# Hiroshiba/realtime-yukarin

Hardware: NVIDIA H100
Metric: chunks_per_s_0.3s_24kHz_encode_stage1_stage2_vocode (higher is better)
Workload: dtype f64 (WORLD analysis / synthesis, SPTK), f16 operands / f32 accumulate: stage-2 k4 layers on wgmma, stage-1 k4 layers on mma.sync inside the one-launch cluster kernel; f32 CUDA cores (3x3 / k3 edge layers)

## Files before the change

### realtime_yukarin_b200/csrc/api.cu

```cuda
#include <math.h>
#include <stddef.h>
#include <stdlib.h>
#include <string.h>
#include <mutex>
#include <algorithm>
#include <vector>

#include "../../include/ryk.h"
#include "conv.h"
#include "drift.h"
#include "engine.h"
#include "fft.cuh"
#include "features.h"
#include "synth.h"
#include "unet.h"

namespace ryk {

static thread_local std::string g_err;
void set_error(const std::string& msg) { g_err = msg; }

void fft_fill_twiddles(double2* t) {
  for (int k = 0; k < kTwiddleN / 2; ++k) t[k] = make_double2(cos(2.0 * kPi * k / kTwiddleN), -sin(2.0 * kPi * k / kTwiddleN));
}
// ... 109 lines not shown
  if (voiced[i]) v = has_stats ? (float)exp((log((double)f0[i]) - mu_i) / sd_i * sd_t + mu_t) : f0[i];
  out[i] = v;
}

static int stage1_plan_for(Engine* e, int Tp, UNetPlan** plan) {
  RYK_CHECK(e->voices[0]->stage1 != nullptr, "stage-1 model not loaded");
  return unet_get_plan(e, e->voices[0]->stage1, 1, 1, Tp, e->precision, plan);
}
static int stage2_plan_for(Engine* e, int Tp, UNetPlan** plan) {
  RYK_CHECK(e->voices[0]->stage2 != nullptr, "stage-2 model not loaded");
  return unet_get_plan(e, e->voices[0]->stage2, 1, Tp, 512, e->precision, plan);
}

static int voice_for_update(Engine* e, int id, Voice** out) {
  Voice* v = engine_voice(e, id);
  RYK_CHECK(v != nullptr, "no such voice");
  RYK_CHECK(id == 0 || v->users == 0, "voice is in use by a session or group: destroy them before changing its models or statistics");
  *out = v;
  return 0;
}

}

using namespace ryk;

static Engine* E(ryk_engine* e) { return &e->impl; }

extern "C" {

int ryk_abi_version(void) { return 1; }
const char* ryk_last_error(void) { return g_err.c_str(); }

int ryk_engine_create(int device, ryk_engine** out) {
  RYK_CHECK(out != nullptr, "null out pointer");
  setenv("CUDA_DEVICE_MAX_CONNECTIONS", "32", 0);
  int count = 0;
  RYK_CUDA(cudaGetDeviceCount(&count));
  RYK_CHECK(count > 0 && device < count, "no such CUDA device (libryk has no CPU fallback)");
  RYK_CUDA(cudaSetDevice(device));
  cudaDeviceProp prop;
  RYK_CUDA(cudaGetDeviceProperties(&prop, device));
  RYK_CHECK(prop.major == 9 && prop.minor == 0, "libryk is built for sm_90a (H100) only");
  ryk_engine* h = new ryk_engine();
  Engine* e = &h->impl;
  e->device = device;
  e->voices.push_back(new Voice());
  RYK_CUDA(cudaStreamCreateWithFlags(&e->stream, cudaStreamNonBlocking));
  std::vector<double2> tw(kTwiddleN / 2);
  fft_fill_twiddles(tw.data());
  RYK_CUDA(cudaMalloc(&e->d_twiddle, sizeof(double2) * tw.size()));
  RYK_CUDA(cudaMemcpy(e->d_twiddle, tw.data(), sizeof(double2) * tw.size(), cudaMemcpyHostToDevice));
  if (analysis_kernels_init()) return -1;
  if (tc_init()) return -1;
  if (s1_fused_init()) return -1;
  RYK_CUDA(cudaMalloc(&e->d_colmin, sizeof(float) * kColminFloats));
  RYK_CUDA(cudaMalloc(&e->d_launches, sizeof(*e->d_launches)));
  RYK_CUDA(cudaMemset(e->d_launches, 0, sizeof(*e->d_launches)));
  *out = h;
  return 0;
}

int ryk_engine_destroy(ryk_engine* h) {
  if (!h) return 0;
  Engine* e = E(h);
  cudaSetDevice(e->device);
  cudaStreamSynchronize(e->stream);
  drift_destroy_all(e);
  reblock_destroy_all(e);
  session_destroy_all(e);
  crepe_destroy();
  for (auto& kv : e->dio_plans) dio_plan_free(kv.second);
  for (Voice* v : e->voices) voice_free(v);
  for (Synth* s : e->synths) synth_destroy(s);
  for (auto& kv : e->sptk) { cudaFree(kv.second.d_G); cudaFree(kv.second.d_H); }
  void* ptrs[] = {e->d_colmin, e->d_launches, e->d_twiddle, e->d_jump, e->d_scratch};
  for (void* p : ptrs) if (p) cudaFree(p);
  if (e->h_pinned) cudaFreeHost(e->h_pinned);
  cudaStreamDestroy(e->stream);
  delete h;
  return 0;
}

int ryk_engine_set_precision(ryk_engine* h, int mode) {
  RYK_CHECK(mode == 0 || mode == 1, "precision mode must be 0 (fp32) or 1 (fp16 tensor core)");
  E(h)->precision = mode;
  return 0;
}
int ryk_engine_get_precision(ryk_engine* h) { return E(h)->precision; }
int ryk_engine_set_stage1_fused(ryk_engine* h, int enable) { E(h)->s1_fused = enable != 0; return s1_fused_cluster_size(); }
long long ryk_engine_launch_count(ryk_engine* h) {
  Engine* e = E(h);
  unsigned long long device_count = 0;
  RYK_CUDA(cudaSetDevice(e->device));
  RYK_CUDA(cudaDeviceSynchronize());
  RYK_CUDA(cudaMemcpy(&device_count, e->d_launches, sizeof(device_count), cudaMemcpyDeviceToHost));
  return e->launches + (long long)device_count;
}
int ryk_engine_synchronize(ryk_engine* h) { RYK_CUDA(cudaSetDevice(E(h)->device)); RYK_CUDA(cudaDeviceSynchronize()); return 0; }

int ryk_engine_profile(ryk_engine* h, int enable) { E(h)->profile = enable != 0; return 0; }
int ryk_engine_profile_read2(ryk_engine* h, double* stage2_ms_total, double* stage2_ms_union, int* stage2_runs) {
  Engine* e = E(h);
  RYK_CUDA(cudaDeviceSynchronize());
  double tot = 0.0, uni = 0.0;
  std::vector<std::pair<double, double>> iv;
  for (auto& pr : e->prof_events) {
// ... 693 lines not shown
```

### realtime_yukarin_b200/csrc/conv.h

```cpp
#pragma once
#include <cuda.h>

#include "common.cuh"

namespace ryk {

enum Act { ACT_NONE = 0, ACT_LEAKY = 1, ACT_RELU = 2 };
enum DType { DT_F32 = 0, DT_F16 = 1 };

constexpr int kMaxGroupVoices = 8;
constexpr int kMaxGroupBatch = 64;

struct LayerWeights {
  const float* w[kMaxGroupVoices];
  const float* scale[kMaxGroupVoices];
  const float* shift[kMaxGroupVoices];
  float host_scale[kMaxGroupVoices], host_shift[kMaxGroupVoices];
  uint8_t voice_of[kMaxGroupBatch];
};
__host__ __device__ inline int item_voice(const LayerWeights& wt, int b) { return b < kMaxGroupBatch ? wt.voice_of[b] : 0; }
struct TcWeightMaps { CUtensorMap m[kMaxGroupVoices]; };

struct ConvLayer {
  int transposed = 0;
  int B = 1, Hin = 1, Win = 1, Hout = 1, Wout = 1;
  int C0 = 0, C1 = 0, Cout = 0;
  int KH = 1, KW = 1, SH = 1, SW = 1, PH = 0, PW = 0;
  int act = ACT_NONE;
  int band_y0 = 0, band_y1 = 0;
  int skip_y0 = 0, skip_y1 = 0;
  int run_y0 = 0, run_y1 = 0;
  const void* in0 = nullptr; const void* in1 = nullptr; int in_dtype = DT_F32;
  void* out = nullptr; int out_dtype = DT_F32;
  int n_voices = 1;
  LayerWeights wt = {};
  bool host_scale_valid = false;
  const __half* w_tc[kMaxGroupVoices] = {};
  const __half* w_frag = nullptr;
  int ksplit = 1;
  int ksplit_tiles = 0;
  CUtensorMap tmA0, tmA1, tmO;
  TcWeightMaps tmB;
  int tile_w = 0, tile_h = 0;
  int block_n = 0;
  bool tc_ready = false;
};

inline int layer_class_rows(const ConvLayer& L) { return L.transposed ? L.Hin : L.Hout; }
inline int layer_band_end(const ConvLayer& L) { return L.band_y1 > 0 ? L.band_y1 : layer_class_rows(L); }
inline void layer_band_out_rows(const ConvLayer& L, int* r0, int* r1) {
  const int s = L.transposed ? L.SH : 1;
  *r0 = L.band_y0 * s;
  *r1 = layer_band_end(L) * s < L.Hout ? layer_band_end(L) * s : L.Hout;
}

int pack_weights_direct(const float* d_w_chainer, int transposed, int Cin, int Cout, int KH, int KW, float* d_out, cudaStream_t st);
int pack_weights_tc(const float* d_w_chainer, int transposed, int Cin, int Cout, int KH, int KW, int SH, int SW, __half* d_out, cudaStream_t st);

int conv_direct_run(const ConvLayer& L, cudaStream_t st);
bool conv_direct_band_supported(const ConvLayer& L);
bool conv_direct_cin1(const ConvLayer& L);
constexpr int kCin1Rows = 8;
bool conv_direct_per_item_weights(const ConvLayer& L);

bool tc_layer_eligible(const ConvLayer& L);
int tc_init();
int tc_layer_prepare(ConvLayer& L, int num_sms);
int tc_layer_weight_maps(ConvLayer& L);
int conv_tc_run(const ConvLayer& L, cudaStream_t st);
int tc_tile_rows(const ConvLayer& L);
int tc_tile_count(const ConvLayer& L);

int s1_pack_weights(const float* d_w_chainer, int transposed, int Cin, int Cout, __half* d_out, cudaStream_t st);
int s1_fused_init();
int s1_fused_cluster_size();

}
```

### realtime_yukarin_b200/csrc/conv_direct.cu

```cuda
#include "conv.h"

namespace ryk {

template <typename T> __device__ inline float ld_act(const T* p);
template <> __device__ inline float ld_act<float>(const float* p) { return *p; }
template <> __device__ inline float ld_act<__half>(const __half* p) { return __half2float(*p); }
template <typename T> __device__ inline void st_act(T* p, float v);
template <> __device__ inline void st_act<float>(float* p, float v) { *p = v; }
template <> __device__ inline void st_act<__half>(__half* p, float v) { *p = __float2half_rn(v); }

struct DirectParams {
  int transposed, B, Hin, Win, Hout, Wout, C0, C1, Cout, KH, KW, SH, SW, PH, PW, act;
  int classH, classW;
  int Hc, Wc;
  const void* in0; const void* in1; void* out;
  const float* w; const float* scale; const float* shift;
};

template <typename TIn, typename TOut>
__global__ void __launch_bounds__(256) k_conv_direct(DirectParams p) {
  constexpr int BM = 64, BN = 64, BK = 16;
  __shared__ float As[BK][BM + 4];
  __shared__ float Bs[BK][BN + 4];
  __shared__ int pix_b[BM], pix_y[BM], pix_x[BM];
  const int Cin = p.C0 + p.C1;
  const int cls = blockIdx.z;
  const int py = cls / p.classW, px = cls % p.classW;
  const int npix = p.B * p.Hc * p.Wc;
  const int m0 = blockIdx.x * BM, n0 = blockIdx.y * BN;
  const int tid = threadIdx.x, ty = tid >> 4, tx = tid & 15;
  if (tid < BM) {
    int q = m0 + tid;
    if (q < npix) {
      int b = q / (p.Hc * p.Wc);
      int r = q - b * p.Hc * p.Wc;
      int my = r / p.Wc, mx = r - my * p.Wc;
      pix_b[tid] = b; pix_y[tid] = my * p.classH + py; pix_x[tid] = mx * p.classW + px;
    } else {
      pix_b[tid] = -1; pix_y[tid] = 0; pix_x[tid] = 0;
    }
  }
  __syncthreads();
  float acc[4][4];
#pragma unroll
  for (int i = 0; i < 4; ++i)
#pragma unroll
    for (int j = 0; j < 4; ++j) acc[i][j] = 0.f;

  const int a_pix = tid >> 2, a_c4 = (tid & 3) * 4;
  const int b_k = tid >> 4, b_n4 = (tid & 15) * 4;
  const TIn* in0 = (const TIn*)p.in0;
  const TIn* in1 = (const TIn*)p.in1;

// ... 39 lines not shown
#pragma unroll
          for (int i = 0; i < 4; ++i)
#pragma unroll
            for (int j = 0; j < 4; ++j) acc[i][j] = fmaf(a[i], b[j], acc[i][j]);
        }
        __syncthreads();
      }
    }
  }
  TOut* out = (TOut*)p.out;
#pragma unroll
  for (int i = 0; i < 4; ++i) {
    int pl = ty * 4 + i;
    int b = pix_b[pl];
    if (b < 0) continue;
    size_t obase = ((size_t)(b * p.Hout + pix_y[pl]) * p.Wout + pix_x[pl]) * p.Cout;
#pragma unroll
    for (int j = 0; j < 4; ++j) {
      int n = n0 + tx * 4 + j;
      if (n >= p.Cout) continue;
      float v = acc[i][j] * p.scale[n] + p.shift[n];
      if (p.act == ACT_LEAKY) v = v > 0.f ? v : 0.2f * v;
      else if (p.act == ACT_RELU) v = v > 0.f ? v : 0.f;
      st_act<TOut>(out + obase + n, v);
    }
  }
}

static int conv_direct_generic(const ConvLayer& L, cudaStream_t st) {
  DirectParams p;
  p.transposed = L.transposed; p.B = L.B; p.Hin = L.Hin; p.Win = L.Win; p.Hout = L.Hout; p.Wout = L.Wout;
  p.C0 = L.C0; p.C1 = L.C1; p.Cout = L.Cout; p.KH = L.KH; p.KW = L.KW; p.SH = L.SH; p.SW = L.SW; p.PH = L.PH; p.PW = L.PW;
  p.act = L.act;
  p.classH = L.transposed ? L.SH : 1; p.classW = L.transposed ? L.SW : 1;
  RYK_CHECK(L.Hout % p.classH == 0 && L.Wout % p.classW == 0, "transposed conv output must be a multiple of the stride");
  p.Hc = L.Hout / p.classH; p.Wc = L.Wout / p.classW;
  p.in0 = L.in0; p.in1 = L.in1; p.out = L.out; p.w = L.wt.w[0]; p.scale = L.wt.scale[0]; p.shift = L.wt.shift[0];
  RYK_CHECK(p.w && p.scale && p.shift && L.in0 && L.out, "direct conv layer is missing a device pointer");
  int npix = L.B * p.Hc * p.Wc;
  dim3 grid((npix + 63) / 64, (L.Cout + 63) / 64, p.classH * p.classW);
  if (L.in_dtype == DT_F32 && L.out_dtype == DT_F32) k_conv_direct<float, float><<<grid, 256, 0, st>>>(p);
  else if (L.in_dtype == DT_F32 && L.out_dtype == DT_F16) k_conv_direct<float, __half><<<grid, 256, 0, st>>>(p);
  else if (L.in_dtype == DT_F16 && L.out_dtype == DT_F16) k_conv_direct<__half, __half><<<grid, 256, 0, st>>>(p);
  else k_conv_direct<__half, float><<<grid, 256, 0, st>>>(p);
  RYK_CUDA(cudaGetLastError());
  return 0;
}



template <typename TOut>
__global__ void __launch_bounds__(256) k_conv3x3_cin1(const float* __restrict__ in, const __grid_constant__ LayerWeights wt, int act,
                                                     int B, int H, int W, int Cout, int skip_b0, int skip_nb, TOut* __restrict__ out) {
  constexpr int kRows = kCin1Rows;
  const int groups = Cout >> 3;
  const int g = threadIdx.x % groups, xl = threadIdx.x / groups;
  const int x = blockIdx.x * 32 + xl;
  const int y0 = (blockIdx.y + (blockIdx.y >= skip_b0 ? skip_nb : 0)) * kRows;
  const int b = blockIdx.z;
  const int voice = item_voice(wt, b);
  const float* __restrict__ w = wt.w[voice];
  const float* __restrict__ scale = wt.scale[voice];
  const float* __restrict__ shift = wt.shift[voice];
  float wr[9][8], sc[8], sh[8];
#pragma unroll
  for (int t = 0; t < 9; ++t)
#pragma unroll
    for (int j = 0; j < 8; ++j) wr[t][j] = __ldg(w + t * Cout + g * 8 + j);
#pragma unroll
  for (int j = 0; j < 8; ++j) { sc[j] = __ldg(scale + g * 8 + j); sh[j] = __ldg(shift + g * 8 + j); }
  if (x >= W) return;
  const float* base = in + (size_t)b * H * W;
  auto ld = [&](int yy, int xx) -> float { return (yy >= 0 && yy < H && xx >= 0 && xx < W) ? __ldg(base + (size_t)yy * W + xx) : 0.f; };
  float r0[3], r1[3], r2[3];
#pragma unroll
  for (int d = 0; d < 3; ++d) { r0[d] = ld(y0 - 1, x + d - 1); r1[d] = ld(y0, x + d - 1); }
  for (int yy = 0; yy < kRows; ++yy) {
    const int y = y0 + yy;
    if (y >= H) break;
#pragma unroll
    for (int d = 0; d < 3; ++d) r2[d] = ld(y + 1, x + d - 1);
    float o[8];
#pragma unroll
    for (int j = 0; j < 8; ++j) {
      float a = 0.f;
#pragma unroll
      for (int d = 0; d < 3; ++d) { a = fmaf(r0[d], wr[d][j], a); a = fmaf(r1[d], wr[3 + d][j], a); a = fmaf(r2[d], wr[6 + d][j], a); }
      a = a * sc[j] + sh[j];
      if (act == ACT_LEAKY) a = a > 0.f ? a : 0.2f * a; else if (act == ACT_RELU) a = fmaxf(a, 0.f);
      o[j] = a;
    }
    TOut* dst = out + (((size_t)b * H + y) * W + x) * Cout + g * 8;
    if constexpr (sizeof(TOut) == 2) {
      __half2 h0 = __floats2half2_rn(o[0], o[1]), h1 = __floats2half2_rn(o[2], o[3]), h2 = __floats2half2_rn(o[4], o[5]), h3 = __floats2half2_rn(o[6], o[7]);
      *reinterpret_cast<uint4*>(dst) = make_uint4(*reinterpret_cast<uint32_t*>(&h0), *reinterpret_cast<uint32_t*>(&h1),
                                                  *reinterpret_cast<uint32_t*>(&h2), *reinterpret_cast<uint32_t*>(&h3));
    } else {
      *reinterpret_cast<float4*>(dst) = make_float4(o[0], o[1], o[2], o[3]);
      *reinterpret_cast<float4*>(dst + 4) = make_float4(o[4], o[5], o[6], o[7]);
    }
#pragma unroll
    for (int d = 0; d < 3; ++d) { r0[d] = r1[d]; r1[d] = r2[d]; }
  }
}

__global__ void __launch_bounds__(256) k_conv3x3_cout1_h(const __half* __restrict__ in0, const __half* __restrict__ in1,
                                                        const __grid_constant__ LayerWeights weights, int act,
                                                        int B, int H, int W, int y0, float* __restrict__ out) {
  const int lane = threadIdx.x & 31, warp = threadIdx.x >> 5;
  const int x0 = (blockIdx.x * 8 + warp) * 8;
  const int y = y0 + blockIdx.y, b = blockIdx.z;
  const int voice = item_voice(weights, b);
  const float* __restrict__ w = weights.w[voice];
  const float scale = weights.host_scale[voice], shift = weights.host_shift[voice];
  if (x0 >= W) return;
  const __half* src = lane < 16 ? in0 : in1;
  const int c = (lane & 15) * 4;
  float wt[9][4];
#pragma unroll
  for (int t = 0; t < 9; ++t)
#pragma unroll
    for (int j = 0; j < 4; ++j) wt[t][j] = __ldg(w + t * 128 + (lane < 16 ? 0 : 64) + c + j);
  float acc[8];
#pragma unroll
  for (int q = 0; q < 8; ++q) acc[q] = 0.f;
#pragma unroll
  for (int dy = 0; dy < 3; ++dy) {
    const int iy = y + dy - 1;
    if (iy < 0 || iy >= H) continue;
    uint2 raw[10];
#pragma unroll
    for (int i = 0; i < 10; ++i) {
      const int ix = x0 + i - 1;
      raw[i] = (ix >= 0 && ix < W) ? __ldg(reinterpret_cast<const uint2*>(src + (((size_t)b * H + iy) * W + ix) * 64 + c)) : make_uint2(0u, 0u);
    }
#pragma unroll
    for (int i = 0; i < 10; ++i) {
      const float2 f01 = __half22float2(*reinterpret_cast<__half2*>(&raw[i].x)), f23 = __half22float2(*reinterpret_cast<__half2*>(&raw[i].y));
#pragma unroll
      for (int dx = 0; dx < 3; ++dx) {
        const int q = i - dx;
        if (q < 0 || q >= 8) continue;
        const float* wv = wt[dy * 3 + dx];
        acc[q] = fmaf(f01.x, wv[0], acc[q]); acc[q] = fmaf(f01.y, wv[1], acc[q]);
        acc[q] = fmaf(f23.x, wv[2], acc[q]); acc[q] = fmaf(f23.y, wv[3], acc[q]);
      }
    }
  }
#pragma unroll
  for (int q = 0; q < 8; ++q) {
#pragma unroll
    for (int o = 16; o > 0; o >>= 1) acc[q] += __shfl_xor_sync(0xffffffffu, acc[q], o);
  }
  if (lane < 8) {
    float a = acc[0];
#pragma unroll
    for (int q = 1; q < 8; ++q) a = lane == q ? acc[q] : a;
    const int x = x0 + lane;
    if (x < W) {
      a = a * scale + shift;
      if (act == ACT_LEAKY) a = a > 0.f ? a : 0.2f * a; else if (act == ACT_RELU) a = fmaxf(a, 0.f);
      out[((size_t)b * H + y) * W + x] = a;
    }
  }
}

__global__ void __launch_bounds__(256) k_conv1d_k3_small(const __half* __restrict__ in0, const __half* __restrict__ in1,
                                                        const float* __restrict__ w , const float* __restrict__ scale,
                                                        const float* __restrict__ shift, int act, int B, int W, int Cout, float* __restrict__ out) {
  const int lane = threadIdx.x & 31;
  const int pos = blockIdx.x * 8 + (threadIdx.x >> 5);
  if (pos >= B * W) return;
  const int b = pos / W, x = pos - b * W;
  const __half* src = lane < 16 ? in0 : in1;
  const int c = (lane & 15) * 4, cg = lane * 4;
  float xin[3][4];
#pragma unroll
  for (int t = 0; t < 3; ++t) {
    const int ix = x + t - 1;
    uint2 raw = make_uint2(0u, 0u);
    if (ix >= 0 && ix < W) raw = __ldg(reinterpret_cast<const uint2*>(src + ((size_t)b * W + ix) * 64 + c));
    const float2 f01 = __half22float2(*reinterpret_cast<__half2*>(&raw.x)), f23 = __half22float2(*reinterpret_cast<__half2*>(&raw.y));
    xin[t][0] = f01.x; xin[t][1] = f01.y; xin[t][2] = f23.x; xin[t][3] = f23.y;
  }
  float mine = 0.f;
  for (int co = 0; co < Cout; ++co) {
    float a = 0.f;
#pragma unroll
    for (int t = 0; t < 3; ++t)
#pragma unroll
      for (int j = 0; j < 4; ++j) a = fmaf(xin[t][j], __ldg(w + ((size_t)t * 128 + cg + j) * Cout + co), a);
#pragma unroll
    for (int o = 16; o > 0; o >>= 1) a += __shfl_xor_sync(0xffffffffu, a, o);
    if (lane == co) mine = a;
  }
  if (lane < Cout) {
    float a = mine * __ldg(scale + lane) + __ldg(shift + lane);
    if (act == ACT_LEAKY) a = a > 0.f ? a : 0.2f * a; else if (act == ACT_RELU) a = fmaxf(a, 0.f);
    out[(size_t)pos * Cout + lane] = a;
  }
}

__global__ void k_read2(const float* a, const float* b, float* out) { out[0] = a[0]; out[1] = b[0]; }

bool conv_direct_band_supported(const ConvLayer& L) {
  return !L.transposed && L.KH == 3 && L.KW == 3 && L.SH == 1 && L.SW == 1 && L.PH == 1 && L.PW == 1 && L.Cout == 1 && L.C0 == 64 &&
         L.C1 == 64 && L.in_dtype == DT_F16 && L.out_dtype == DT_F32 && L.host_scale_valid;
}

bool conv_direct_cin1(const ConvLayer& L) {
  return !L.transposed && L.KH == 3 && L.KW == 3 && L.SH == 1 && L.SW == 1 && L.PH == 1 && L.PW == 1 && L.C0 == 1 && L.C1 == 0 &&
         L.in_dtype == DT_F32 && L.Cout % 8 == 0 && L.Cout <= 64;
}

bool conv_direct_per_item_weights(const ConvLayer& L) { return conv_direct_cin1(L) || conv_direct_band_supported(L); }

int conv_direct_run(const ConvLayer& L, cudaStream_t st) {
  const bool cout1_h = conv_direct_band_supported(L);
  const bool cin1 = conv_direct_cin1(L);
  RYK_CHECK(L.n_voices == 1 || cout1_h || cin1, "of the CUDA-core kernels only the stage-2 edge layers take weights per batch item");
  RYK_CHECK(cout1_h || (L.band_y0 == 0 && L.band_y1 == 0), "of the CUDA-core kernels only the Cout = 1 3x3 kernel computes a row band");
  RYK_CHECK(cin1 || L.skip_y1 == 0, "of the CUDA-core kernels only the Cin = 1 3x3 kernel skips a padded tail");
  if (!L.transposed && L.KH == 3 && L.KW == 3 && L.SH == 1 && L.SW == 1 && L.PH == 1 && L.PW == 1) {
    if (cin1) {
      RYK_CHECK(L.skip_y0 % kCin1Rows == 0 && L.skip_y1 % kCin1Rows == 0 && L.skip_y0 <= L.skip_y1 && L.skip_y1 <= L.Hout,
                "skipped rows are not whole row blocks of the first layer");
      const int skip_b0 = L.skip_y0 / kCin1Rows, skip_nb = (L.skip_y1 - L.skip_y0) / kCin1Rows;
      dim3 grid((L.Win + 31) / 32, (L.Hin + kCin1Rows - 1) / kCin1Rows - skip_nb, L.B);
      int threads = 32 * (L.Cout / 8);
      if (L.out_dtype == DT_F16)
        k_conv3x3_cin1<__half><<<grid, threads, 0, st>>>((const float*)L.in0, L.wt, L.act, L.B, L.Hin, L.Win, L.Cout, skip_b0, skip_nb, (__half*)L.out);
      else
        k_conv3x3_cin1<float><<<grid, threads, 0, st>>>((const float*)L.in0, L.wt, L.act, L.B, L.Hin, L.Win, L.Cout, skip_b0, skip_nb, (float*)L.out);
      RYK_CUDA(cudaGetLastError());
      return 0;
    }
    if (cout1_h) {
      dim3 blocks((L.Win + 63) / 64, layer_band_end(L) - L.band_y0, L.B);
      k_conv3x3_cout1_h<<<blocks, 256, 0, st>>>((const __half*)L.in0, (const __half*)L.in1, L.wt, L.act,
                                                L.B, L.Hin, L.Win, L.band_y0, (float*)L.out);
      RYK_CUDA(cudaGetLastError());
      return 0;
    }
  }
  if (!L.transposed && L.KH == 1 && L.KW == 3 && L.SW == 1 && L.PW == 1 && L.Hin == 1 && L.C0 == 64 && L.C1 == 64 && L.Cout <= 16 &&
      L.in_dtype == DT_F16 && L.out_dtype == DT_F32) {
    const int npos = L.B * L.Win;
    k_conv1d_k3_small<<<(npos + 7) / 8, 256, 0, st>>>((const __half*)L.in0, (const __half*)L.in1, L.wt.w[0], L.wt.scale[0], L.wt.shift[0], L.act, L.B, L.Win, L.Cout,
                                                     (float*)L.out);
    RYK_CUDA(cudaGetLastError());
    return 0;
  }
  return conv_direct_generic(L, st);
}

__global__ void k_pack_direct(const float* __restrict__ w, int transposed, int Cin, int Cout, int KH, int KW, float* __restrict__ out) {
  size_t total = (size_t)KH * KW * Cin * Cout;
  for (size_t i = blockIdx.x * (size_t)blockDim.x + threadIdx.x; i < total; i += (size_t)gridDim.x * blockDim.x) {
    int n = i % Cout; size_t r = i / Cout;
    int c = r % Cin; r /= Cin;
    int kx = r % KW; int ky = r / KW;
    size_t src = transposed ? (((size_t)c * Cout + n) * KH + ky) * KW + kx : (((size_t)n * Cin + c) * KH + ky) * KW + kx;
    out[i] = w[src];
  }
}

int pack_weights_direct(const float* d_w, int transposed, int Cin, int Cout, int KH, int KW, float* d_out, cudaStream_t st) {
  k_pack_direct<<<256, 256, 0, st>>>(d_w, transposed, Cin, Cout, KH, KW, d_out);
  RYK_CUDA(cudaGetLastError());
  return 0;
}

__global__ void k_pack_tc(const float* __restrict__ w, int transposed, int Cin, int Cout, int KH, int KW, int SH, int SW,
                          __half* __restrict__ out) {
  size_t total = (size_t)KH * KW * Cin * Cout;
  for (size_t i = blockIdx.x * (size_t)blockDim.x + threadIdx.x; i < total; i += (size_t)gridDim.x * blockDim.x) {
    if (!transposed) {
      size_t K = (size_t)KH * KW * Cin;
      int n = i / K; size_t k = i % K;
      int tap = k / Cin, c = k % Cin;
      int ky = tap / KW, kx = tap % KW;
      out[i] = __float2half_rn(w[(((size_t)n * Cin + c) * KH + ky) * KW + kx]);
    } else {
      int th = KH / SH, tw = KW / SW;
      size_t K = (size_t)th * tw * Cin;
      size_t per_cls = K * Cout;
      int cls = i / per_cls; size_t r = i % per_cls;
      int n = r / K; size_t k = r % K;
      int tap = k / Cin, c = k % Cin;
      int dy = tap / tw, dx = tap % tw, py = cls / SW, px = cls % SW;
      int ky = SH == 2 ? 3 - 2 * dy - py : 0, kx = SW == 2 ? 3 - 2 * dx - px : 0;
      out[i] = __float2half_rn(w[(((size_t)c * Cout + n) * KH + ky) * KW + kx]);
    }
// ... 11 lines not shown
```

### realtime_yukarin_b200/csrc/conv_tc.cu

```cuda
#include <cuda.h>
#include <cudaTypedefs.h>

#include "conv.h"
#include "tc_ptx.cuh"

namespace ryk {

struct TcParams {
  int transposed, B, Hout, Wout, Cout;
  int Hc, Wc;
  int tile_w, tile_h, tiles_w, tiles_h;
  int th0;
  int skip_t0, skip_tn;
  int run_y0, run_y1;
  int chunks0, chunks1;
  int taps_w, ntaps;
  int sh, sw, ph, pw;
  int classes_w;
  int ksplit, chunks_per_split;
  int act;
  LayerWeights wt;
  __half* out;
};

// ... 294 lines not shown

static void tc_geometry(const ConvLayer& L, int num_sms, int* tile_w, int* tile_h, int* block_n, int* ksplit) {
  int tw, th;
  tc_tile_shape(L, &tw, &th);
  int bn = L.Cout >= 128 ? 128 : 64;
  int tiles = L.ksplit_tiles > 0 ? L.ksplit_tiles : tc_tile_count(L);
  int ntaps = L.transposed ? (L.KH / L.SH) * (L.KW / L.SW) : L.KH * L.KW;
  int total_chunks = ntaps * (L.C0 + L.C1) / kBlockK;
  int ks = 1;
  int slots = num_sms * 2;
  if (tiles < slots) {
    constexpr int kMinChunks = 8;
    ks = slots / tiles;
    if (ks > total_chunks / kMinChunks) ks = total_chunks / kMinChunks;
    if (ks > kMaxSplits) ks = kMaxSplits;
    if (ks < 1) ks = 1;
    while (ks > 1 && tiles > g_clusters[ks]) --ks;
    int cps = (total_chunks + ks - 1) / ks;
    ks = (total_chunks + cps - 1) / cps;
  }
  *tile_w = tw; *tile_h = th; *block_n = bn; *ksplit = ks;
}

int tc_layer_weight_maps(ConvLayer& L) {
  RYK_CHECK(L.n_voices >= 1 && L.n_voices <= kMaxGroupVoices, "a layer holds 1..8 voices");
  const int classes = L.transposed ? L.SH * L.SW : 1;
  const int ntaps = L.transposed ? (L.KH / L.SH) * (L.KW / L.SW) : L.KH * L.KW;
  const size_t K = (size_t)ntaps * (L.C0 + L.C1), rows = (size_t)classes * L.Cout;
  for (int v = 0; v < L.n_voices; ++v) {
    RYK_CHECK(L.w_tc[v] != nullptr, "tensor-core layer without packed weights for one of its voices");
    if (make_weight_map(&L.tmB.m[v], L.w_tc[v], K, rows, L.block_n)) return -1;
  }
  for (int v = L.n_voices; v < kMaxGroupVoices; ++v) L.tmB.m[v] = L.tmB.m[0];
  return 0;
}

int tc_layer_prepare(ConvLayer& L, int num_sms) {
  RYK_CHECK(g_encode != nullptr, "tc_init() was not called");
  RYK_CHECK(tc_layer_eligible(L), "layer is not eligible for the tensor-core path");
  tc_geometry(L, num_sms, &L.tile_w, &L.tile_h, &L.block_n, &L.ksplit);
  int stw = L.transposed ? 1 : L.SW, sth = L.transposed ? 1 : L.SH;
  if (make_act_map(&L.tmA0, L.in0, L.C0, L.Win, L.Hin, L.B, L.tile_w, L.tile_h, stw, sth)) return -1;
  if (L.C1 > 0) { if (make_act_map(&L.tmA1, L.in1, L.C1, L.Win, L.Hin, L.B, L.tile_w, L.tile_h, stw, sth)) return -1; }
  else L.tmA1 = L.tmA0;
  if (tc_layer_weight_maps(L)) return -1;
  if (make_act_map(&L.tmO, L.out, L.Cout, L.Wout, L.Hout, L.B, L.tile_w, L.tile_h, L.transposed ? L.SW : 1, L.transposed ? L.SH : 1)) return -1;
  RYK_CHECK(L.band_y0 >= 0 && L.band_y0 % L.tile_h == 0 && L.band_y0 < layer_band_end(L) && layer_band_end(L) <= layer_class_rows(L) &&
            (layer_band_end(L) % L.tile_h == 0 || layer_band_end(L) == layer_class_rows(L)), "row band is not a range of whole tile rows");
  RYK_CHECK(L.skip_y1 == 0 || (!L.transposed && L.skip_y0 % L.tile_h == 0 && L.skip_y1 % L.tile_h == 0 && L.band_y0 <= L.skip_y0 &&
                               L.skip_y0 < L.skip_y1 && L.skip_y1 <= layer_band_end(L)),
            "skipped rows are not a range of whole tile rows inside the band of a convolution");
  L.tc_ready = true;
  return 0;
}

template <typename... KArgs, typename... Args>
static cudaError_t launch_pdl(void (*kernel)(KArgs...), dim3 grid, dim3 block, size_t smem, cudaStream_t st, int cluster_z, Args&&... args) {
  cudaLaunchConfig_t cfg = {};
  cfg.gridDim = grid; cfg.blockDim = block; cfg.dynamicSmemBytes = smem; cfg.stream = st;
  cudaLaunchAttribute attr[2];
  attr[0].id = cudaLaunchAttributeProgrammaticStreamSerialization; attr[0].val.programmaticStreamSerializationAllowed = 1;
  attr[1].id = cudaLaunchAttributeClusterDimension; attr[1].val.clusterDim.x = 1; attr[1].val.clusterDim.y = 1; attr[1].val.clusterDim.z = cluster_z;
  cfg.attrs = attr; cfg.numAttrs = cluster_z > 1 ? 2 : 1;
  return cudaLaunchKernelEx(&cfg, kernel, static_cast<KArgs>(args)...);
}

int conv_tc_run(const ConvLayer& L, cudaStream_t st) {
  RYK_CHECK(L.tc_ready, "tc layer not prepared");
  TcParams p;
  p.transposed = L.transposed; p.B = L.B; p.Hout = L.Hout; p.Wout = L.Wout; p.Cout = L.Cout;
  p.Hc = L.transposed ? L.Hin : L.Hout; p.Wc = L.transposed ? L.Win : L.Wout;
  p.tile_w = L.tile_w; p.tile_h = L.tile_h;
  p.skip_t0 = L.skip_y0 / L.tile_h; p.skip_tn = (L.skip_y1 - L.skip_y0) / L.tile_h;
  p.tiles_w = (p.Wc + L.tile_w - 1) / L.tile_w; p.tiles_h = (layer_band_end(L) - L.band_y0 + L.tile_h - 1) / L.tile_h - p.skip_tn;
  p.th0 = L.band_y0 / L.tile_h;
  p.run_y0 = L.run_y0; p.run_y1 = L.run_y1;
  p.chunks0 = L.C0 / kBlockK; p.chunks1 = L.C1 / kBlockK;
  p.taps_w = L.transposed ? L.KW / L.SW : L.KW;
  p.ntaps = L.transposed ? (L.KH / L.SH) * (L.KW / L.SW) : L.KH * L.KW;
  p.sh = L.SH; p.sw = L.SW; p.ph = L.PH; p.pw = L.PW;
  p.classes_w = L.transposed ? L.SW : 1;
  const int classes = L.transposed ? L.SH * L.SW : 1;
  p.ksplit = L.ksplit;
  int total_chunks = p.ntaps * (p.chunks0 + p.chunks1);
  p.chunks_per_split = (total_chunks + L.ksplit - 1) / L.ksplit;
  p.act = L.act; p.wt = L.wt;
  p.out = (__half*)L.out;
  dim3 grid(L.B * p.tiles_w * p.tiles_h, L.Cout / L.block_n, classes * L.ksplit);
  if (L.block_n == 128) RYK_CUDA(launch_pdl(RYK_TC_N128, grid, dim3(kTcThreads), tc_smem_bytes<128, 3>(), st, L.ksplit, L.tmA0, L.tmA1, L.tmB, L.tmO, p));
  else RYK_CUDA(launch_pdl(RYK_TC_N64, grid, dim3(kTcThreads), tc_smem_bytes<64, 4>(), st, L.ksplit, L.tmA0, L.tmA1, L.tmB, L.tmO, p));
  RYK_CUDA(cudaGetLastError());
  return 0;
}

}
```

### realtime_yukarin_b200/csrc/tc_ptx.cuh

```cuda
#pragma once
#include <cuda.h>
#include <stdint.h>

namespace ryk {

constexpr int kBlockM = 128;
constexpr int kBlockK = 64;
constexpr int kMmaK = 16;
constexpr int kTcConsumers = 256;
constexpr int kTcThreads = kTcConsumers + 32;

__device__ __forceinline__ uint32_t smem_u32(const void* p) { return (uint32_t)__cvta_generic_to_shared(p); }

__device__ __forceinline__ void pdl_trigger() { asm volatile("griddepcontrol.launch_dependents;" ::: "memory"); }
__device__ __forceinline__ void pdl_wait() { asm volatile("griddepcontrol.wait;" ::: "memory"); }

__device__ __forceinline__ bool elect_one() {
  uint32_t pred;
  asm volatile("{\n\t.reg .pred p;\n\telect.sync _|p, 0xffffffff;\n\tselp.u32 %0, 1, 0, p;\n\t}" : "=r"(pred));
  return pred != 0;
}

__device__ __forceinline__ void mbar_init(uint64_t* bar, uint32_t count) {
  asm volatile("mbarrier.init.shared::cta.b64 [%0], %1;" ::"r"(smem_u32(bar)), "r"(count));
}
__device__ __forceinline__ void mbar_expect_tx(uint64_t* bar, uint32_t bytes) {
  asm volatile("mbarrier.arrive.expect_tx.shared::cta.b64 _, [%0], %1;" ::"r"(smem_u32(bar)), "r"(bytes) : "memory");
}
__device__ __forceinline__ void mbar_arrive(uint64_t* bar) {
  asm volatile("mbarrier.arrive.shared::cta.b64 _, [%0];" ::"r"(smem_u32(bar)) : "memory");
}
__device__ __forceinline__ void mbar_wait(uint64_t* bar, uint32_t parity) {
  asm volatile(
      "{\n\t"
      ".reg .pred p;\n\t"
      "WAIT_LOOP:\n\t"
      "mbarrier.try_wait.parity.shared::cta.b64 p, [%0], %1;\n\t"
      "@p bra WAIT_DONE;\n\t"
      "bra WAIT_LOOP;\n\t"
      "WAIT_DONE:\n\t"
      "}" ::"r"(smem_u32(bar)), "r"(parity) : "memory");
}
__device__ __forceinline__ void tma_load_4d(void* dst, const CUtensorMap* map, uint64_t* bar, int c0, int c1, int c2, int c3) {
  asm volatile(
      "cp.async.bulk.tensor.4d.shared::cluster.global.mbarrier::complete_tx::bytes [%0], [%1, {%3, %4, %5, %6}], [%2];"
      ::"r"(smem_u32(dst)), "l"(map), "r"(smem_u32(bar)), "r"(c0), "r"(c1), "r"(c2), "r"(c3) : "memory");
}
__device__ __forceinline__ void tma_load_2d(void* dst, const CUtensorMap* map, uint64_t* bar, int c0, int c1) {
  asm volatile(
      "cp.async.bulk.tensor.2d.shared::cluster.global.mbarrier::complete_tx::bytes [%0], [%1, {%3, %4}], [%2];"
      ::"r"(smem_u32(dst)), "l"(map), "r"(smem_u32(bar)), "r"(c0), "r"(c1) : "memory");
}
__device__ __forceinline__ void wgmma_fence() { asm volatile("wgmma.fence.sync.aligned;" ::: "memory"); }
__device__ __forceinline__ void wgmma_commit() { asm volatile("wgmma.commit_group.sync.aligned;" ::: "memory"); }
template <int N> __device__ __forceinline__ void wgmma_wait() { asm volatile("wgmma.wait_group.sync.aligned %0;" ::"n"(N) : "memory"); }
template <int R> __device__ __forceinline__ void wgmma_fence_acc(float (&d)[R]) {
#pragma unroll
  for (int i = 0; i < R; ++i) asm volatile("" : "+f"(d[i])::"memory");
}
__device__ __forceinline__ void wgmma_m64n64(float (&d)[32], uint64_t adesc, uint64_t bdesc) {
  asm volatile(
      "{\n\t.reg .pred p;\n\tsetp.ne.b32 p, %34, 0;\n\t"
      "wgmma.mma_async.sync.aligned.m64n64k16.f32.f16.f16 "
      "{%0, %1, %2, %3, %4, %5, %6, %7, %8, %9, %10, %11, %12, %13, %14, %15, %16, %17, %18, %19, %20, %21, %22, %23, %24, %25, %26, %27, %28, %29, %30, %31}, "
      "%32, %33, p, 1, 1, 0, 0;\n\t}"
      : "+f"(d[0]), "+f"(d[1]), "+f"(d[2]), "+f"(d[3]), "+f"(d[4]), "+f"(d[5]), "+f"(d[6]), "+f"(d[7]), "+f"(d[8]), "+f"(d[9]), "+f"(d[10]), "+f"(d[11]), "+f"(d[12]), "+f"(d[13]), "+f"(d[14]), "+f"(d[15]), "+f"(d[16]), "+f"(d[17]), "+f"(d[18]), "+f"(d[19]), "+f"(d[20]), "+f"(d[21]), "+f"(d[22]), "+f"(d[23]), "+f"(d[24]), "+f"(d[25]), "+f"(d[26]), "+f"(d[27]), "+f"(d[28]), "+f"(d[29]), "+f"(d[30]), "+f"(d[31])
      : "l"(adesc), "l"(bdesc), "r"(1));
}
// ... 36 lines not shown
```

Baseline: 2614.

## Launch edge 3x3 convs with PDL and stage their inputs in shared memory

The first (Cin=1) and last (Cout=1) 3x3 direct-conv kernels are now launched with programmatic dependent launch. They trigger dependents early and wait only after loading weights, so they can overlap with the previous kernel's tail. Both kernels now stage their input halo tile in shared memory: the cin1 kernel through a plain load loop, the cout1 kernel through cp.async into dynamic smem. The cout1 kernel also handles four output rows per block instead of one, reusing the staged rows across the vertical taps. This trades repeated global loads for a larger shared-memory footprint and fewer blocks.

After: 2649, median of 6. +1.4%, better.

```diff
diff --git a/realtime_yukarin_b200/csrc/api.cu b/realtime_yukarin_b200/csrc/api.cu
--- a/realtime_yukarin_b200/csrc/api.cu
+++ b/realtime_yukarin_b200/csrc/api.cu
@@ -185,6 +185,7 @@
   RYK_CUDA(cudaMemcpy(e->d_twiddle, tw.data(), sizeof(double2) * tw.size(), cudaMemcpyHostToDevice));
   if (analysis_kernels_init()) return -1;
   if (tc_init()) return -1;
+  if (conv_direct_init()) return -1;
   if (s1_fused_init()) return -1;
   RYK_CUDA(cudaMalloc(&e->d_colmin, sizeof(float) * kColminFloats));
   RYK_CUDA(cudaMalloc(&e->d_launches, sizeof(*e->d_launches)));
diff --git a/realtime_yukarin_b200/csrc/conv.h b/realtime_yukarin_b200/csrc/conv.h
--- a/realtime_yukarin_b200/csrc/conv.h
+++ b/realtime_yukarin_b200/csrc/conv.h
@@ -57,6 +57,7 @@
 int pack_weights_direct(const float* d_w_chainer, int transposed, int Cin, int Cout, int KH, int KW, float* d_out, cudaStream_t st);
 int pack_weights_tc(const float* d_w_chainer, int transposed, int Cin, int Cout, int KH, int KW, int SH, int SW, __half* d_out, cudaStream_t st);
 
+int conv_direct_init();
 int conv_direct_run(const ConvLayer& L, cudaStream_t st);
 bool conv_direct_band_supported(const ConvLayer& L);
 bool conv_direct_cin1(const ConvLayer& L);
diff --git a/realtime_yukarin_b200/csrc/conv_direct.cu b/realtime_yukarin_b200/csrc/conv_direct.cu
--- a/realtime_yukarin_b200/csrc/conv_direct.cu
+++ b/realtime_yukarin_b200/csrc/conv_direct.cu
@@ -1,4 +1,5 @@
 #include "conv.h"
+#include "pdl.cuh"
 
 namespace ryk {
 
@@ -144,10 +145,11 @@
 template <typename TOut>
 __global__ void __launch_bounds__(256) k_conv3x3_cin1(const float* __restrict__ in, const __grid_constant__ LayerWeights wt, int act,
                                                      int B, int H, int W, int Cout, int skip_b0, int skip_nb, TOut* __restrict__ out) {
+  pdl_trigger();
   constexpr int kRows = kCin1Rows;
   const int groups = Cout >> 3;
   const int g = threadIdx.x % groups, xl = threadIdx.x / groups;
-  const int x = blockIdx.x * 32 + xl;
+  const int x0 = blockIdx.x * 32, x = x0 + xl;
   const int y0 = (blockIdx.y + (blockIdx.y >= skip_b0 ? skip_nb : 0)) * kRows;
   const int b = blockIdx.z;
   const int voice = item_voice(wt, b);
@@ -161,17 +163,23 @@
     for (int j = 0; j < 8; ++j) wr[t][j] = __ldg(w + t * Cout + g * 8 + j);
 #pragma unroll
   for (int j = 0; j < 8; ++j) { sc[j] = __ldg(scale + g * 8 + j); sh[j] = __ldg(shift + g * 8 + j); }
+  pdl_wait();
+  __shared__ float s_in[kRows + 2][34];
+  const float* base = in + (size_t)b * H * W;
+  for (int i = threadIdx.x; i < (kRows + 2) * 34; i += blockDim.x) {
+    const int r = i / 34, c = i - r * 34, yy = y0 + r - 1, xx = x0 + c - 1;
+    s_in[r][c] = (yy >= 0 && yy < H && xx >= 0 && xx < W) ? __ldg(base + (size_t)yy * W + xx) : 0.f;
+  }
+  __syncthreads();
   if (x >= W) return;
-  const float* base = in + (size_t)b * H * W;
-  auto ld = [&](int yy, int xx) -> float { return (yy >= 0 && yy < H && xx >= 0 && xx < W) ? __ldg(base + (size_t)yy * W + xx) : 0.f; };
   float r0[3], r1[3], r2[3];
 #pragma unroll
-  for (int d = 0; d < 3; ++d) { r0[d] = ld(y0 - 1, x + d - 1); r1[d] = ld(y0, x + d - 1); }
+  for (int d = 0; d < 3; ++d) { r0[d] = s_in[0][xl + d]; r1[d] = s_in[1][xl + d]; }
   for (int yy = 0; yy < kRows; ++yy) {
     const int y = y0 + yy;
     if (y >= H) break;
 #pragma unroll
-    for (int d = 0; d < 3; ++d) r2[d] = ld(y + 1, x + d - 1);
+    for (int d = 0; d < 3; ++d) r2[d] = s_in[yy + 2][xl + d];
     float o[8];
 #pragma unroll
     for (int j = 0; j < 8; ++j) {
@@ -196,63 +204,90 @@
   }
 }
 
+constexpr int kCout1Rows = 4;
+constexpr int kCout1Px = 64;
+constexpr size_t kCout1Smem = (size_t)(kCout1Rows + 2) * (kCout1Px + 2) * 256;
+
+__device__ __forceinline__ void cp_async16(uint32_t dst, const void* src, bool valid) {
+  asm volatile("cp.async.cg.shared.global [%0], [%1], 16, %2;" ::"r"(dst), "l"(src), "r"(valid ? 16 : 0) : "memory");
+}
+
 __global__ void __launch_bounds__(256) k_conv3x3_cout1_h(const __half* __restrict__ in0, const __half* __restrict__ in1,
                                                         const __grid_constant__ LayerWeights weights, int act,
-                                                        int B, int H, int W, int y0, float* __restrict__ out) {
+                                                        int B, int H, int W, int y0, int y1, float* __restrict__ out) {
+  extern __shared__ __align__(16) uint8_t s_in[];
+  pdl_trigger();
   const int lane = threadIdx.x & 31, warp = threadIdx.x >> 5;
-  const int x0 = (blockIdx.x * 8 + warp) * 8;
-  const int y = y0 + blockIdx.y, b = blockIdx.z;
+  const int bx0 = blockIdx.x * kCout1Px;
+  const int ya = y0 + blockIdx.y * kCout1Rows;
+  const int rows = min(kCout1Rows, y1 - ya);
+  const int b = blockIdx.z;
   const int voice = item_voice(weights, b);
   const float* __restrict__ w = weights.w[voice];
   const float scale = weights.host_scale[voice], shift = weights.host_shift[voice];
-  if (x0 >= W) return;
-  const __half* src = lane < 16 ? in0 : in1;
   const int c = (lane & 15) * 4;
   float wt[9][4];
 #pragma unroll
   for (int t = 0; t < 9; ++t)
 #pragma unroll
     for (int j = 0; j < 4; ++j) wt[t][j] = __ldg(w + t * 128 + (lane < 16 ? 0 : 64) + c + j);
-  float acc[8];
-#pragma unroll
-  for (int q = 0; q < 8; ++q) acc[q] = 0.f;
-#pragma unroll
-  for (int dy = 0; dy < 3; ++dy) {
-    const int iy = y + dy - 1;
-    if (iy < 0 || iy >= H) continue;
-    uint2 raw[10];
-#pragma unroll
-    for (int i = 0; i < 10; ++i) {
-      const int ix = x0 + i - 1;
-      raw[i] = (ix >= 0 && ix < W) ? __ldg(reinterpret_cast<const uint2*>(src + (((size_t)b * H + iy) * W + ix) * 64 + c)) : make_uint2(0u, 0u);
-    }
-#pragma unroll
-    for (int i = 0; i < 10; ++i) {
-      const float2 f01 = __half22float2(*reinterpret_cast<__half2*>(&raw[i].x)), f23 = __half22float2(*reinterpret_cast<__half2*>(&raw[i].y));
-#pragma unroll
-      for (int dx = 0; dx < 3; ++dx) {
-        const int q = i - dx;
-        if (q < 0 || q >= 8) continue;
-        const float* wv = wt[dy * 3 + dx];
-        acc[q] = fmaf(f01.x, wv[0], acc[q]); acc[q] = fmaf(f01.y, wv[1], acc[q]);
-        acc[q] = fmaf(f23.x, wv[2], acc[q]); acc[q] = fmaf(f23.y, wv[3], acc[q]);
+  pdl_wait();
+  {
+    const uint32_t s_base = (uint32_t)__cvta_generic_to_shared(s_in);
+    const int pieces = (rows + 2) * (kCout1Px + 2) * 16;
+    for (int q = threadIdx.x; q < pieces; q += blockDim.x) {
+      const int k = q & 15, px = (q >> 4) % (kCout1Px + 2), r = (q >> 4) / (kCout1Px + 2);
+      const int iy = ya + r - 1, ix = bx0 + px - 1;
+      const bool ok = iy >= 0 && iy < H && ix >= 0 && ix < W;
+      const __half* src = (k < 8 ? in0 : in1) + (ok ? (((size_t)b * H + iy) * W + ix) * 64 + (k & 7) * 8 : 0);
+      cp_async16(s_base + (uint32_t)q * 16, src, ok);
+    }
+    asm volatile("cp.async.wait_all;" ::: "memory");
+  }
+  __syncthreads();
+  const int x0 = bx0 + warp * 8;
+  if (x0 >= W) return;
+  for (int rr = 0; rr < rows; ++rr) {
+    const int y = ya + rr;
+    float acc[8];
+#pragma unroll
+    for (int q = 0; q < 8; ++q) acc[q] = 0.f;
+#pragma unroll
+    for (int dy = 0; dy < 3; ++dy) {
+      const int iy = y + dy - 1;
+      if (iy < 0 || iy >= H) continue;
+      const uint2* row = reinterpret_cast<const uint2*>(s_in + ((size_t)(rr + dy) * (kCout1Px + 2) + warp * 8) * 256) + lane;
+      uint2 raw[10];
+#pragma unroll
+      for (int i = 0; i < 10; ++i) raw[i] = row[i * 32];
+#pragma unroll
+      for (int i = 0; i < 10; ++i) {
+        const float2 f01 = __half22float2(*reinterpret_cast<__half2*>(&raw[i].x)), f23 = __half22float2(*reinterpret_cast<__half2*>(&raw[i].y));
+#pragma unroll
+        for (int dx = 0; dx < 3; ++dx) {
+          const int q = i - dx;
+          if (q < 0 || q >= 8) continue;
+          const float* wv = wt[dy * 3 + dx];
+          acc[q] = fmaf(f01.x, wv[0], acc[q]); acc[q] = fmaf(f01.y, wv[1], acc[q]);
+          acc[q] = fmaf(f23.x, wv[2], acc[q]); acc[q] = fmaf(f23.y, wv[3], acc[q]);
+        }
       }
     }
-  }
-#pragma unroll
-  for (int q = 0; q < 8; ++q) {
-#pragma unroll
-    for (int o = 16; o > 0; o >>= 1) acc[q] += __shfl_xor_sync(0xffffffffu, acc[q], o);
-  }
-  if (lane < 8) {
-    float a = acc[0];
-#pragma unroll
-    for (int q = 1; q < 8; ++q) a = lane == q ? acc[q] : a;
-    const int x = x0 + lane;
-    if (x < W) {
-      a = a * scale + shift;
-      if (act == ACT_LEAKY) a = a > 0.f ? a : 0.2f * a; else if (act == ACT_RELU) a = fmaxf(a, 0.f);
-      out[((size_t)b * H + y) * W + x] = a;
+#pragma unroll
+    for (int q = 0; q < 8; ++q) {
+#pragma unroll
+      for (int o = 16; o > 0; o >>= 1) acc[q] += __shfl_xor_sync(0xffffffffu, acc[q], o);
+    }
+    if (lane < 8) {
+      float a = acc[0];
+#pragma unroll
+      for (int q = 1; q < 8; ++q) a = lane == q ? acc[q] : a;
+      const int x = x0 + lane;
+      if (x < W) {
+        a = a * scale + shift;
+        if (act == ACT_LEAKY) a = a > 0.f ? a : 0.2f * a; else if (act == ACT_RELU) a = fmaxf(a, 0.f);
+        out[((size_t)b * H + y) * W + x] = a;
+      }
     }
   }
 }
@@ -306,6 +341,11 @@
 }
 
 bool conv_direct_per_item_weights(const ConvLayer& L) { return conv_direct_cin1(L) || conv_direct_band_supported(L); }
+
+int conv_direct_init() {
+  RYK_CUDA(cudaFuncSetAttribute(k_conv3x3_cout1_h, cudaFuncAttributeMaxDynamicSharedMemorySize, (int)kCout1Smem));
+  return 0;
+}
 
 int conv_direct_run(const ConvLayer& L, cudaStream_t st) {
   const bool cout1_h = conv_direct_band_supported(L);
@@ -318,19 +358,22 @@
       RYK_CHECK(L.skip_y0 % kCin1Rows == 0 && L.skip_y1 % kCin1Rows == 0 && L.skip_y0 <= L.skip_y1 && L.skip_y1 <= L.Hout,
                 "skipped rows are not whole row blocks of the first layer");
       const int skip_b0 = L.skip_y0 / kCin1Rows, skip_nb = (L.skip_y1 - L.skip_y0) / kCin1Rows;
-      dim3 grid((L.Win + 31) / 32, (L.Hin + kCin1Rows - 1) / kCin1Rows - skip_nb, L.B);
-      int threads = 32 * (L.Cout / 8);
+      const dim3 grid((L.Win + 31) / 32, (L.Hin + kCin1Rows - 1) / kCin1Rows - skip_nb, L.B);
+      const int threads = 32 * (L.Cout / 8);
       if (L.out_dtype == DT_F16)
-        k_conv3x3_cin1<__half><<<grid, threads, 0, st>>>((const float*)L.in0, L.wt, L.act, L.B, L.Hin, L.Win, L.Cout, skip_b0, skip_nb, (__half*)L.out);
+        RYK_CUDA(launch_pdl(k_conv3x3_cin1<__half>, grid, dim3(threads), 0, st, 1, (const float*)L.in0, L.wt, L.act, L.B, L.Hin, L.Win, L.Cout,
+                            skip_b0, skip_nb, (__half*)L.out));
       else
-        k_conv3x3_cin1<float><<<grid, threads, 0, st>>>((const float*)L.in0, L.wt, L.act, L.B, L.Hin, L.Win, L.Cout, skip_b0, skip_nb, (float*)L.out);
+        RYK_CUDA(launch_pdl(k_conv3x3_cin1<float>, grid, dim3(threads), 0, st, 1, (const float*)L.in0, L.wt, L.act, L.B, L.Hin, L.Win, L.Cout,
+                            skip_b0, skip_nb, (float*)L.out));
       RYK_CUDA(cudaGetLastError());
       return 0;
     }
     if (cout1_h) {
-      dim3 blocks((L.Win + 63) / 64, layer_band_end(L) - L.band_y0, L.B);
-      k_conv3x3_cout1_h<<<blocks, 256, 0, st>>>((const __half*)L.in0, (const __half*)L.in1, L.wt, L.act,
-                                                L.B, L.Hin, L.Win, L.band_y0, (float*)L.out);
+      const int y0 = L.band_y0, y1 = layer_band_end(L);
+      const dim3 grid((L.Win + kCout1Px - 1) / kCout1Px, (y1 - y0 + kCout1Rows - 1) / kCout1Rows, L.B);
+      RYK_CUDA(launch_pdl(k_conv3x3_cout1_h, grid, dim3(256), kCout1Smem, st, 1, (const __half*)L.in0, (const __half*)L.in1, L.wt, L.act,
+                          L.B, L.Hin, L.Win, y0, y1, (float*)L.out));
       RYK_CUDA(cudaGetLastError());
       return 0;
     }
diff --git a/realtime_yukarin_b200/csrc/conv_tc.cu b/realtime_yukarin_b200/csrc/conv_tc.cu
--- a/realtime_yukarin_b200/csrc/conv_tc.cu
+++ b/realtime_yukarin_b200/csrc/conv_tc.cu
@@ -370,17 +370,6 @@
             "skipped rows are not a range of whole tile rows inside the band of a convolution");
   L.tc_ready = true;
   return 0;
-}
-
-template <typename... KArgs, typename... Args>
-static cudaError_t launch_pdl(void (*kernel)(KArgs...), dim3 grid, dim3 block, size_t smem, cudaStream_t st, int cluster_z, Args&&... args) {
-  cudaLaunchConfig_t cfg = {};
-  cfg.gridDim = grid; cfg.blockDim = block; cfg.dynamicSmemBytes = smem; cfg.stream = st;
-  cudaLaunchAttribute attr[2];
-  attr[0].id = cudaLaunchAttributeProgrammaticStreamSerialization; attr[0].val.programmaticStreamSerializationAllowed = 1;
-  attr[1].id = cudaLaunchAttributeClusterDimension; attr[1].val.clusterDim.x = 1; attr[1].val.clusterDim.y = 1; attr[1].val.clusterDim.z = cluster_z;
-  cfg.attrs = attr; cfg.numAttrs = cluster_z > 1 ? 2 : 1;
-  return cudaLaunchKernelEx(&cfg, kernel, static_cast<KArgs>(args)...);
 }
 
 int conv_tc_run(const ConvLayer& L, cudaStream_t st) {
diff --git a/realtime_yukarin_b200/csrc/pdl.cuh b/realtime_yukarin_b200/csrc/pdl.cuh
--- /dev/null
+++ b/realtime_yukarin_b200/csrc/pdl.cuh
@@ -0,0 +1,20 @@
+#pragma once
+#include <cuda_runtime.h>
+
+namespace ryk {
+
+__device__ __forceinline__ void pdl_trigger() { asm volatile("griddepcontrol.launch_dependents;" ::: "memory"); }
+__device__ __forceinline__ void pdl_wait() { asm volatile("griddepcontrol.wait;" ::: "memory"); }
+
+template <typename... KArgs, typename... Args>
+cudaError_t launch_pdl(void (*kernel)(KArgs...), dim3 grid, dim3 block, size_t smem, cudaStream_t st, int cluster_z, Args&&... args) {
+  cudaLaunchConfig_t cfg = {};
+  cfg.gridDim = grid; cfg.blockDim = block; cfg.dynamicSmemBytes = smem; cfg.stream = st;
+  cudaLaunchAttribute attr[2];
+  attr[0].id = cudaLaunchAttributeProgrammaticStreamSerialization; attr[0].val.programmaticStreamSerializationAllowed = 1;
+  attr[1].id = cudaLaunchAttributeClusterDimension; attr[1].val.clusterDim.x = 1; attr[1].val.clusterDim.y = 1; attr[1].val.clusterDim.z = cluster_z;
+  cfg.attrs = attr; cfg.numAttrs = cluster_z > 1 ? 2 : 1;
+  return cudaLaunchKernelEx(&cfg, kernel, static_cast<KArgs>(args)...);
+}
+
+}
diff --git a/realtime_yukarin_b200/csrc/tc_ptx.cuh b/realtime_yukarin_b200/csrc/tc_ptx.cuh
--- a/realtime_yukarin_b200/csrc/tc_ptx.cuh
+++ b/realtime_yukarin_b200/csrc/tc_ptx.cuh
@@ -1,6 +1,8 @@
 #pragma once
 #include <cuda.h>
 #include <stdint.h>
+
+#include "pdl.cuh"
 
 namespace ryk {
 
@@ -11,9 +13,6 @@
 constexpr int kTcThreads = kTcConsumers + 32;
 
 __device__ __forceinline__ uint32_t smem_u32(const void* p) { return (uint32_t)__cvta_generic_to_shared(p); }
-
-__device__ __forceinline__ void pdl_trigger() { asm volatile("griddepcontrol.launch_dependents;" ::: "memory"); }
-__device__ __forceinline__ void pdl_wait() { asm volatile("griddepcontrol.wait;" ::: "memory"); }
 
 __device__ __forceinline__ bool elect_one() {
   uint32_t pred;
```
